# alibaba/EasyRec

Hardware: NVIDIA H100
Metric: samples_per_sec (higher is better)
Workload: dtype f32

## Files before the change

### easyrec_b200/csrc/embedding_bwd.cu

```cuda
#include "common.cuh"
#include "scan.cuh"
#include "slots.cuh"
#include "sort.cuh"
#include "bucket_bwd.cuh"

namespace er {

struct CBufs {
  const float* p[ER_MAX_BUFS];
};

constexpr int kLongRun = 64;
constexpr int kBatch = 4;
constexpr int kChunk = 512;

struct BwdArgs {
  float* table;
  float* state0;
  float* state1;
  int dim;
  int row_stride;
  uint32_t sentinel;
  const uint32_t* keys;
  const uint32_t* vals;
  const uint64_t* pairs;
  int64_t n;
  const float* weights;
  const int32_t* seg_ids;
  const er_slot_t* slots;
  int n_slots;
  CBufs gbufs;
  const float* seg_scale;
  er_opt_t opt;
  float lr_t;
  const float* hyper;
  int64_t* uniq_rows;
  float* uniq_grads;
  const int32_t* head_rank;
  int32_t* counters;
  int4* long_list;
  int32_t* run_done;
  int2* chunk_list;
  float* partials;
  const int64_t* or_rows;
  float* or_partials;
  int32_t* or_tickets;
  int or_chunks;
  int main_ctas;
};

__device__ __forceinline__ const float* grad_src(const BwdArgs& a, const SlotView& sv, uint32_t l,
                                                 float* coef) {
  const int32_t s = a.seg_ids ? a.seg_ids[l] : (int32_t)l;
  const SlotLite sl = slot_lite(sv, slot_of(sv, s));
  float c = (a.weights && !slot_unit_weights(sl)) ? a.weights[l] : 1.0f;
  if (a.seg_scale) c = __fmul_rn(c, a.seg_scale[s]);
  *coef = c;
  return a.gbufs.p[sl.misc & 0xff] + (int64_t)(s - sl.seg_begin) * sl.out_stride + sl.out_col;
}

struct Hyper {
  float lr, lr_t, grad_scale;
};

__device__ __forceinline__ Hyper load_hyper(const er_opt_t& o, float lr_t_arg, const float* __restrict__ hyper) {
  Hyper h;
  if (hyper) {
    h.lr = __ldg(hyper + ER_HYPER_LR);
    h.grad_scale = __ldg(hyper + ER_HYPER_GRAD_SCALE);
    h.lr_t = h.lr;
    if (o.kind == ER_OPT_LAZY_ADAM || o.kind == ER_OPT_ADAM_ROWS)
      h.lr_t = adam_lr_t_of(h.lr, __ldg(hyper + ER_HYPER_BETA1_POWER), __ldg(hyper + ER_HYPER_BETA2_POWER));
  } else {
    h.lr = o.lr;
    h.lr_t = lr_t_arg;
    h.grad_scale = o.grad_scale;
  }
  return h;
}

__device__ __forceinline__ void upd_one(const BwdArgs& a, const Hyper& h, float g, float& w, float& s0, float& s1) {
  switch (a.opt.kind) {
    case ER_OPT_ADAGRAD: {
      s0 = __fadd_rn(s0, __fmul_rn(g, g));
      w = __fsub_rn(w, __fmul_rn(__fmul_rn(h.lr, g), __frsqrt_rn(s0)));
      break;
    }
    case ER_OPT_LAZY_ADAM:
    case ER_OPT_ADAM_ROWS: {
      s0 = __fadd_rn(__fmul_rn(g, 1.0f - a.opt.beta1), __fmul_rn(s0, a.opt.beta1));
      s1 = __fadd_rn(__fmul_rn(__fmul_rn(g, g), 1.0f - a.opt.beta2), __fmul_rn(s1, a.opt.beta2));
      w = __fadd_rn(w, __fdiv_rn(__fmul_rn(-h.lr_t, s0), __fadd_rn(__fsqrt_rn(s1), a.opt.eps)));
      break;
    }
    case ER_OPT_MOMENTUM: {
      s0 = __fadd_rn(__fmul_rn(s0, a.opt.beta1), g);
      w = __fsub_rn(w, __fmul_rn(h.lr, s0));
      break;
    }
    default:
      w = __fsub_rn(w, __fmul_rn(h.lr, g));
  }
}

__device__ __forceinline__ void f4_fma_sep(float4& g, const float4& v, float c) {
  g.x = __fadd_rn(g.x, __fmul_rn(v.x, c));
  g.y = __fadd_rn(g.y, __fmul_rn(v.y, c));
  g.z = __fadd_rn(g.z, __fmul_rn(v.z, c));
  g.w = __fadd_rn(g.w, __fmul_rn(v.w, c));
}
__device__ __forceinline__ void f4_acc(float4& g, const float4& v) {
  g.x = __fadd_rn(g.x, v.x);
  g.y = __fadd_rn(g.y, v.y);
  g.z = __fadd_rn(g.z, v.z);
  g.w = __fadd_rn(g.w, v.w);
}

__device__ __forceinline__ float4 f4_scale1(const float4& v, float c) {
  return make_float4(__fmul_rn(v.x, c), __fmul_rn(v.y, c), __fmul_rn(v.z, c), __fmul_rn(v.w, c));
}

struct RowRegs {
  float4 w, s0, s1;
};

__device__ __forceinline__ RowRegs load_row(const BwdArgs& a, uint32_t row, int lane) {
  RowRegs r;
  r.w = r.s0 = r.s1 = make_float4(0.f, 0.f, 0.f, 0.f);
  if (!a.table) return r;
  const int64_t off = (int64_t)row * a.row_stride;
  r.w = reinterpret_cast<const float4*>(a.table + off)[lane];
  if (a.state0) r.s0 = reinterpret_cast<const float4*>(a.state0 + off)[lane];
  if (a.state1) r.s1 = reinterpret_cast<const float4*>(a.state1 + off)[lane];
  return r;
}

__device__ __forceinline__ void apply_row_vec(const BwdArgs& a, uint32_t row, int lane, float4 g,
                                              int64_t head_pos, RowRegs r) {
  const Hyper h = load_hyper(a.opt, a.lr_t, a.hyper);
  g.x = __fmul_rn(g.x, h.grad_scale);
  g.y = __fmul_rn(g.y, h.grad_scale);
  g.z = __fmul_rn(g.z, h.grad_scale);
  g.w = __fmul_rn(g.w, h.grad_scale);
  if (a.uniq_rows) {
    const int32_t u = a.head_rank[head_pos];
    if (lane == 0) a.uniq_rows[u] = (int64_t)row;
    reinterpret_cast<float4*>(a.uniq_grads + (int64_t)u * a.dim)[lane] = g;
  }
  if (!a.table) return;
  upd_one(a, h, g.x, r.w.x, r.s0.x, r.s1.x);
  upd_one(a, h, g.y, r.w.y, r.s0.y, r.s1.y);
  upd_one(a, h, g.z, r.w.z, r.s0.z, r.s1.z);
  upd_one(a, h, g.w, r.w.w, r.s0.w, r.s1.w);
  const int64_t off = (int64_t)row * a.row_stride;
  reinterpret_cast<float4*>(a.table + off)[lane] = r.w;
  if (a.state0) reinterpret_cast<float4*>(a.state0 + off)[lane] = r.s0;
  if (a.state1) reinterpret_cast<float4*>(a.state1 + off)[lane] = r.s1;
}

__device__ __forceinline__ void apply_scalar(const BwdArgs& a, uint32_t key, int c, float g,
                                             int64_t head_pos) {
  const Hyper h = load_hyper(a.opt, a.lr_t, a.hyper);
  g = __fmul_rn(g, h.grad_scale);
  if (a.uniq_rows) {
    const int32_t u = a.head_rank[head_pos];
    if (c == 0) a.uniq_rows[u] = (int64_t)key;
    a.uniq_grads[(int64_t)u * a.dim + c] = g;
  }
  if (!a.table) return;
  const int64_t off = (int64_t)key * a.row_stride + c;
  float w = a.table[off];
  float s0 = a.state0 ? a.state0[off] : 0.f;
  float s1 = a.state1 ? a.state1[off] : 0.f;
  upd_one(a, h, g, w, s0, s1);
  a.table[off] = w;
  if (a.state0) a.state0[off] = s0;
  if (a.state1) a.state1[off] = s1;
}

__device__ __forceinline__ int64_t run_end(const uint32_t* __restrict__ keys, int64_t lo, int64_t n,
                                           uint32_t key) {
  int64_t step = 1, hi = lo + 1;
  while (hi < n && keys[hi] == key) {
    lo = hi;
    step <<= 1;
    hi = lo + step;
  }
  if (hi > n) hi = n;
  while (hi - lo > 1) {
    const int64_t mid = (lo + hi) >> 1;
    if (keys[mid] == key)
      lo = mid;
    else
      hi = mid;
  }
  return hi;
}

__device__ __forceinline__ void enqueue_run(const BwdArgs& a, int64_t start, int len) {
  const int nch = (len + kChunk - 1) / kChunk;
  const int q = atomicAdd(&a.counters[0], 1);
  const int c0 = atomicAdd(&a.counters[1], nch);
  a.long_list[q] = make_int4((int)start, len, c0, nch);
  a.run_done[q] = 0;
  for (int c = 0; c < nch; ++c) a.chunk_list[c0 + c] = make_int2(q, c);
}

__device__ __forceinline__ void enqueue_long(const BwdArgs& a, int64_t start, int64_t j, uint32_t key) {
  enqueue_run(a, start, (int)(run_end(a.keys, j, a.n, key) - start));
}

__shared__ __align__(16) float s_or_part[1024];
__shared__ int s_or_last;
__shared__ long long s_or_row;

__device__ __forceinline__ int64_t one_row_row(const BwdArgs& a, const er_slot_t& sl) {
  for (int base = 0; base < sl.n_seg; base += blockDim.x) {
    const int e = base + threadIdx.x;
    const int64_t r = e < sl.n_seg ? a.or_rows[(int64_t)sl.seg_begin + e] : -1;
    if (threadIdx.x == 0) s_or_row = -1;
    __syncthreads();
    if (r >= 0) s_or_row = r;
    if (__syncthreads_or(r >= 0)) return s_or_row;
  }
  return -1;
}

template <int LANES>
__device__ __forceinline__ void one_row_cta(const BwdArgs& a, int cta) {
  const int f = cta / a.or_chunks, c_first = cta - f * a.or_chunks;
  const er_slot_t sl = a.slots[f];
  if (sl.bucket_mode != ER_BUCKET_ONE_ROW) return;
  constexpr int L = LANES > 0 ? LANES : 1;
  constexpr int G = 256 / L;
  const int dim = a.dim;
  const int used_chunks = (sl.n_seg + bk::kOneRowChunk - 1) / bk::kOneRowChunk;
  if (c_first >= used_chunks) return;
  const int used_ctas = min(a.or_chunks, used_chunks);
  float* const parts = a.or_partials + ((int64_t)f + sl.seg_begin / bk::kOneRowChunk) * dim;
  const float* gbuf = a.gbufs.p[sl.out_buf];
  if constexpr (LANES > 0) {
    const int grp = threadIdx.x / LANES, lane = threadIdx.x % LANES;
    float4 tot = make_float4(0.f, 0.f, 0.f, 0.f);
    for (int c = c_first; c < used_chunks; c += a.or_chunks) {
      const int s0 = c * bk::kOneRowChunk, s1 = min(sl.n_seg, s0 + bk::kOneRowChunk);
      float4 g = make_float4(0.f, 0.f, 0.f, 0.f);
      constexpr int U = 4;
      for (int e = s0 + grp; e < s1; e += G * U) {
        float4 v[U];
        float coef[U];
        bool use[U];
#pragma unroll
        for (int u = 0; u < U; ++u) {
          const int ee = e + u * G;
          use[u] = false;
          if (ee < s1) {
            const int64_t l = (int64_t)sl.seg_begin + ee;
            use[u] = a.or_rows[l] >= 0;
            coef[u] = a.weights ? a.weights[l] : 1.0f;
            if (a.seg_scale) coef[u] = __fmul_rn(coef[u], a.seg_scale[l]);
            v[u] = reinterpret_cast<const float4*>(gbuf + (int64_t)ee * sl.out_stride + sl.out_col)[lane];
          }
        }
#pragma unroll
        for (int u = 0; u < U; ++u)
          if (use[u]) f4_fma_sep(g, v[u], coef[u]);
      }
      reinterpret_cast<float4*>(s_or_part)[grp * LANES + lane] = g;
      __syncthreads();
      tot = make_float4(0.f, 0.f, 0.f, 0.f);
      if (threadIdx.x < LANES) {
        for (int q = 0; q < G; ++q) f4_acc(tot, reinterpret_cast<float4*>(s_or_part)[q * LANES + threadIdx.x]);
        __stcg(reinterpret_cast<float4*>(parts + (int64_t)c * dim) + threadIdx.x, tot);
      }
      __syncthreads();
    }
    __threadfence();
    __syncthreads();
    if (threadIdx.x == 0) s_or_last = (atomicAdd(&a.or_tickets[f], 1) == used_ctas - 1);
    __syncthreads();
    if (s_or_last) {
      __threadfence();
      for (int base = 0; base < used_chunks; base += G) {
        const int q = base + grp;
        if (q < used_chunks)
          reinterpret_cast<float4*>(s_or_part)[grp * LANES + lane] =
              __ldcg(reinterpret_cast<const float4*>(parts + (int64_t)q * dim) + lane);
        __syncthreads();
        if (threadIdx.x < LANES) {
          if (base == 0) tot = make_float4(0.f, 0.f, 0.f, 0.f);
          const int m = min(G, used_chunks - base);
          for (int q2 = 0; q2 < m; ++q2) f4_acc(tot, reinterpret_cast<float4*>(s_or_part)[q2 * LANES + threadIdx.x]);
        }
        __syncthreads();
      }
      const int64_t row = one_row_row(a, sl);
      if (threadIdx.x < LANES && row >= 0) {
        RowRegs r = load_row(a, (uint32_t)row, threadIdx.x);
        apply_row_vec(a, (uint32_t)row, threadIdx.x, tot, 0, r);
      }
      if (threadIdx.x == 0) a.or_tickets[f] = 0;
    }
  } else {
    for (int c = c_first; c < used_chunks; c += a.or_chunks) {
      const int s0 = c * bk::kOneRowChunk, s1 = min(sl.n_seg, s0 + bk::kOneRowChunk);
      for (int col = 0; col < dim; ++col) {
        float g = 0.f;
        for (int e = s0 + threadIdx.x; e < s1; e += 256) {
          const int64_t l = (int64_t)sl.seg_begin + e;
          if (a.or_rows[l] < 0) continue;
          float coef = a.weights ? a.weights[l] : 1.0f;
          if (a.seg_scale) coef = __fmul_rn(coef, a.seg_scale[l]);
          g = __fadd_rn(g, __fmul_rn(gbuf[(int64_t)e * sl.out_stride + sl.out_col + col], coef));
        }
        s_or_part[threadIdx.x] = g;
        __syncthreads();
        if (threadIdx.x == 0) {
          float tot = 0.f;
          for (int q = 0; q < 256; ++q) tot = __fadd_rn(tot, s_or_part[q]);
          __stcg(parts + (int64_t)c * dim + col, tot);
        }
        __syncthreads();
      }
    }
    __threadfence();
    __syncthreads();
    if (threadIdx.x == 0) s_or_last = (atomicAdd(&a.or_tickets[f], 1) == used_ctas - 1);
    __syncthreads();
    if (s_or_last) {
      __threadfence();
// ... 543 lines not shown
  row.w = row.s0 = row.s1 = make_float4(0.f, 0.f, 0.f, 0.f);
  if (r < R) row = load_row(a, (uint32_t)(sp[s_start[r]] >> 32), lane);
  float4 acc = make_float4(0.f, 0.f, 0.f, 0.f);
  for (int c0 = 0; c0 < n; c0 += S_ENT) {
    const int c1 = min(n, c0 + S_ENT);
    for (int q = threadIdx.x; q < (c1 - c0) * LANES; q += THREADS) {
      const int e = q / LANES;
      const uint32_t pos = (uint32_t)sp[c0 + e];
      if (pos != kDonePos) {
        float coef;
        const float* src = grad_src(a, sv, pos, &coef);
        s_stage[q] = f4_scale1(reinterpret_cast<const float4*>(src)[q % LANES], coef);
      }
    }
    __syncthreads();
    while (r < R && (int)s_start[r] < c1) {
      const int st = s_start[r], en = s_start[r + 1];
      const int lo = max(st, c0), hi = min(en, c1);
      for (int i = lo; i < hi; ++i) f4_acc(acc, s_stage[(i - c0) * LANES + lane]);
      if (en > c1) break;
      const uint32_t key = (uint32_t)(sp[st] >> 32);
      int rn = r + G;
      while (rn < R && run_is_long(s_start, rn)) rn += G;
      RowRegs nxt;
      nxt.w = nxt.s0 = nxt.s1 = make_float4(0.f, 0.f, 0.f, 0.f);
      if (rn < R) nxt = load_row(a, (uint32_t)(sp[s_start[rn]] >> 32), lane);
      apply_row_vec(a, key, lane, acc, 0, row);
      acc = make_float4(0.f, 0.f, 0.f, 0.f);
      row = nxt;
      r = rn;
    }
    __syncthreads();
  }
}

template <int THREADS, typename IdxT>
__device__ __forceinline__ void process_runs_scalar(const BwdArgs& a, const SlotView& sv, uint64_t* sp,
                                                    const IdxT* s_start, int R, float* s_stagef, float* s_partf,
                                                    int* s_coop, int* s_ncoop, int64_t queue_base) {
  const int dim = a.dim;
  if (threadIdx.x == 0) *s_ncoop = 0;
  __syncthreads();
  for (int r = threadIdx.x; r < R; r += THREADS)
    if (run_is_long(s_start, r)) s_coop[atomicAdd(s_ncoop, 1)] = r;
  __syncthreads();
  const int nco = *s_ncoop;
  for (int cc = 0; cc < nco; ++cc) {
    const int r = s_coop[cc];
    const int st = s_start[r], en = s_start[r + 1], len = en - st;
    if (queue_base >= 0 && len > bk::kQueueRun) {
      if (threadIdx.x == 0) enqueue_run(a, queue_base + st, len);
    } else {
      const int chunk = (len + THREADS - 1) / THREADS;
      const int j0 = st + threadIdx.x * chunk, j1 = min(en, j0 + chunk);
      const int used = (len + chunk - 1) / chunk;
      for (int c = 0; c < dim; ++c) {
        float g = 0.f;
        for (int j = j0; j < j1; ++j) {
          float coef;
          const float* src = grad_src(a, sv, (uint32_t)sp[j], &coef);
          g = __fadd_rn(g, __fmul_rn(src[c], coef));
        }
        s_partf[threadIdx.x] = g;
        __syncthreads();
        if (threadIdx.x == 0) {
          float tot = 0.f;
          for (int q = 0; q < used; ++q) tot = __fadd_rn(tot, s_partf[q]);
          apply_scalar(a, (uint32_t)(sp[st] >> 32), c, tot, 0);
        }
        __syncthreads();
      }
    }
    __syncthreads();
    for (int i = st + threadIdx.x; i < en; i += THREADS) sp[i] |= (uint64_t)kDonePos;
  }
  __syncthreads();
  const int n = s_start[R];
  const int S_ENT = max(1, (kStageF4 * 4) / dim);
  for (int cb = 0; cb < dim; cb += THREADS) {
    const int width = min(THREADS, dim - cb);
    const int total = R * width;
    int idx = threadIdx.x;
    float acc = 0.f;
    for (int c0 = 0; c0 < n; c0 += S_ENT) {
      const int c1 = min(n, c0 + S_ENT);
      for (int q = threadIdx.x; q < (c1 - c0) * dim; q += THREADS) {
        const int e = q / dim;
        const uint32_t pos = (uint32_t)sp[c0 + e];
        if (pos != kDonePos) {
          float coef;
          const float* src = grad_src(a, sv, pos, &coef);
          s_stagef[q] = __fmul_rn(src[q - e * dim], coef);
        }
      }
      __syncthreads();
      while (idx < total) {
        const int r = idx / width, c = cb + idx - r * width;
        if (run_is_long(s_start, r)) {
          idx += THREADS;
          continue;
        }
        const int st = s_start[r], en = s_start[r + 1];
        if (st >= c1) break;
        const int lo = max(st, c0), hi = min(en, c1);
        for (int i = lo; i < hi; ++i) acc = __fadd_rn(acc, s_stagef[(i - c0) * dim + c]);
        if (en > c1) break;
        apply_scalar(a, (uint32_t)(sp[st] >> 32), c, acc, 0);
        acc = 0.f;
        idx += THREADS;
      }
      __syncthreads();
    }
  }
}

inline size_t bk_reduce_smem(int n_slots, int cap, int threads) {
  return ((slot_smem_bytes(n_slots) + 15) & ~(size_t)15) + (size_t)cap * 8 + (((size_t)(cap + 1) * 2 + 15) & ~(size_t)15) +
         (size_t)max(kStageF4, threads) * 16 + (size_t)(cap / bk::kCoopRun + 2) * 4 + 64;
}

struct BkSmem {
  uint64_t* pairs;
  uint16_t* start;
  float4* stage;
  float4* part;
  int* coop;
  int* ncoop;
};
__device__ __forceinline__ BkSmem bk_carve(unsigned char* s_raw, int n_slots, int cap, int threads) {
  BkSmem m;
  unsigned char* p = s_raw + ((slot_smem_bytes(n_slots) + 15) & ~(size_t)15);
  m.pairs = reinterpret_cast<uint64_t*>(p); p += (size_t)cap * 8;
  m.start = reinterpret_cast<uint16_t*>(p); p += ((size_t)(cap + 1) * 2 + 15) & ~(size_t)15;
  m.stage = reinterpret_cast<float4*>(p); p += (size_t)max(kStageF4, threads) * 16;
  m.part = m.stage;
  m.coop = reinterpret_cast<int*>(p); p += (size_t)(cap / bk::kCoopRun + 1) * 4;
  m.ncoop = reinterpret_cast<int*>(p);
  return m;
}

__device__ __forceinline__ void cx(uint64_t& lo, uint64_t& hi, bool up) {
  if ((lo > hi) == up) {
    const uint64_t t = lo;
    lo = hi;
    hi = t;
  }
}

template <int LANES>
struct WarpSmem {
  float4 stage[32 * LANES];
  float4 carry[LANES];
  uint32_t keys[32];
};

__device__ __forceinline__ void sort4(uint64_t (&x)[4], int P, int lane) {
  for (int kk = 2; kk <= P; kk <<= 1) {
    for (int j = kk >> 1; j > 0; j >>= 1) {
      if (j == 64) {
        cx(x[0], x[2], ((lane) & kk) == 0);
        cx(x[1], x[3], ((lane + 32) & kk) == 0);
      } else if (j == 32) {
        cx(x[0], x[1], ((lane) & kk) == 0);
        if (P > 64) cx(x[2], x[3], ((lane + 64) & kk) == 0);
      } else {
        const bool lower = (lane & j) == 0;
#pragma unroll
        for (int r = 0; r < 4; ++r) {
          if (r * 32 < P) {
            const uint64_t other = __shfl_xor_sync(0xffffffffu, x[r], j);
            const bool up = ((lane + 32 * r) & kk) == 0;
            if ((x[r] > other) == (lower == up)) x[r] = other;
          }
        }
      }
    }
  }
}

template <int LANES>
__device__ __forceinline__ void warp_bucket_vec(const BwdArgs& a, const SlotView& sv, const BkArgs& k, int b,
                                                WarpSmem<LANES>* ws) {
  constexpr int G = 32 / LANES;
  const int lane = threadIdx.x & 31;
  const int gi = lane / LANES, gl = lane % LANES;
  const int n = k.w.bcnt[b];
  if (n == 0 || n > bk::kWarpCap) return;
  const int64_t off = k.w.boff[b];
  uint64_t x[4];
#pragma unroll
  for (int r = 0; r < 4; ++r) {
    const int q = r * 32 + lane;
    x[r] = q < n ? k.w.pairs[off + q] : ~0ull;
  }
  sort4(x, n <= 32 ? 32 : (n <= 64 ? 64 : 128), lane);
  uint32_t carry_key = 0xFFFFFFFFu;
#pragma unroll
  for (int r = 0; r < 4; ++r) {
    if (r * 32 >= n) break;
    const uint32_t key = (uint32_t)(x[r] >> 32), pos = (uint32_t)x[r];
    const int nv = min(32, n - r * 32);
    const uint32_t next_first = (r < 3 && (r + 1) * 32 < n) ? __shfl_sync(0xffffffffu, (uint32_t)(x[r < 3 ? r + 1 : 3] >> 32), 0)
                                                            : 0xFFFFFFFFu;
    uint32_t prevk = __shfl_up_sync(0xffffffffu, key, 1);
    if (lane == 0) prevk = carry_key;
    const bool is_head = lane < nv && key != prevk;
    const unsigned H = __ballot_sync(0xffffffffu, is_head);
    const int nh = __popc(H);
    ws->keys[lane] = key;
    const float4 open_sum = ws->carry[gl];
    RowRegs row0, row1;
    row0.w = row0.s0 = row0.s1 = row1.w = row1.s0 = row1.s1 = make_float4(0.f, 0.f, 0.f, 0.f);
    {
      const unsigned h0 = __fns(H, 0, gi + 1), h1 = __fns(H, 0, gi + G + 1);
      const uint32_t k0 = __shfl_sync(0xffffffffu, key, h0 & 31), k1 = __shfl_sync(0xffffffffu, key, h1 & 31);
      if (gi < nh) row0 = load_row(a, k0, gl);
      if (gi + G < nh) row1 = load_row(a, k1, gl);
    }
#pragma unroll
    for (int t = 0; t < LANES; ++t) {
      const int e = t * G + gi;
      const uint32_t pe = __shfl_sync(0xffffffffu, pos, e);
      if (e < nv) {
        float coef;
        const float* src = grad_src(a, sv, pe, &coef);
        ws->stage[e * LANES + gl] = f4_scale1(reinterpret_cast<const float4*>(src)[gl], coef);
      }
    }
    __syncwarp();
    const uint32_t lastk = ws->keys[31];
    const bool chunk_open = (nv == 32) && next_first == lastk;
    const int lead = nh ? (__ffs(H) - 1) : nv;
    if (lead > 0 && gi == 0) {
      float4 acc = open_sum;
      for (int i = 0; i < lead; ++i) f4_acc(acc, ws->stage[i * LANES + gl]);
      if (lead == 32 && chunk_open) {
        ws->carry[gl] = acc;
      } else {
        RowRegs row = load_row(a, carry_key, gl);
        apply_row_vec(a, carry_key, gl, acc, 0, row);
      }
    }
    for (int q = gi; q < nh; q += G) {
      const int h = __fns(H, 0, q + 1);
      const unsigned rest = (h == 31) ? 0u : (H >> (h + 1)) << (h + 1);
      const int e_end = rest ? (__ffs(rest) - 1) : nv;
      const uint32_t kh = ws->keys[h];
      float4 acc = make_float4(0.f, 0.f, 0.f, 0.f);
      for (int i = h; i < e_end; ++i) f4_acc(acc, ws->stage[i * LANES + gl]);
      if (e_end == 32 && chunk_open) {
        ws->carry[gl] = acc;
      } else {
        RowRegs row = (q == gi) ? row0 : (q == gi + G) ? row1 : load_row(a, kh, gl);
        apply_row_vec(a, kh, gl, acc, 0, row);
      }
    }
    carry_key = chunk_open ? lastk : 0xFFFFFFFFu;
    __syncwarp();
  }
}

struct WarpSmem1 {
  float stage[32];
  float carry;
  uint32_t keys[32];
};

__device__ __forceinline__ void warp_bucket_scalar(const BwdArgs& a, const SlotView& sv, const BkArgs& k, int b,
                                                   WarpSmem1* ws) {
  const int lane = threadIdx.x & 31;
  const int n = k.w.bcnt[b];
  if (n == 0 || n > bk::kWarpCap) return;
  const int64_t off = k.w.boff[b];
  uint64_t x[4];
#pragma unroll
  for (int r = 0; r < 4; ++r) {
    const int q = r * 32 + lane;
    x[r] = q < n ? k.w.pairs[off + q] : ~0ull;
  }
  sort4(x, n <= 32 ? 32 : (n <= 64 ? 64 : 128), lane);
#pragma unroll 1
  for (int col = 0; col < a.dim; ++col) {
    uint32_t carry_key = 0xFFFFFFFFu;
#pragma unroll
    for (int r = 0; r < 4; ++r) {
      if (r * 32 >= n) break;
      const uint32_t key = (uint32_t)(x[r] >> 32), pos = (uint32_t)x[r];
      const int nv = min(32, n - r * 32);
      const uint32_t next_first = (r < 3 && (r + 1) * 32 < n) ? __shfl_sync(0xffffffffu, (uint32_t)(x[r < 3 ? r + 1 : 3] >> 32), 0)
                                                              : 0xFFFFFFFFu;
      uint32_t prevk = __shfl_up_sync(0xffffffffu, key, 1);
      if (lane == 0) prevk = carry_key;
      const bool is_head = lane < nv && key != prevk;
      const unsigned H = __ballot_sync(0xffffffffu, is_head);
      const int nh = __popc(H);
      ws->keys[lane] = key;
      const float open_sum = ws->carry;
      if (lane < nv) {
        float coef;
        const float* src = grad_src(a, sv, pos, &coef);
        ws->stage[lane] = __fmul_rn(src[col], coef);
      }
      __syncwarp();
      const uint32_t lastk = ws->keys[31];
      const bool chunk_open = (nv == 32) && next_first == lastk;
      const int lead = nh ? (__ffs(H) - 1) : nv;
      if (lead > 0 && lane == 31) {
        float acc = open_sum;
        for (int i = 0; i < lead; ++i) acc = __fadd_rn(acc, ws->stage[i]);
        if (lead == 32 && chunk_open)
          ws->carry = acc;
        else
          apply_scalar(a, carry_key, col, acc, 0);
      }
      if (lane < nh && !(lead > 0 && lane == 31)) {
        const int h = __fns(H, 0, lane + 1);
        const unsigned rest = (h == 31) ? 0u : (H >> (h + 1)) << (h + 1);
        const int e_end = rest ? (__ffs(rest) - 1) : nv;
        float acc = 0.f;
        for (int i = h; i < e_end; ++i) acc = __fadd_rn(acc, ws->stage[i]);
        if (e_end == 32 && chunk_open)
          ws->carry = acc;
        else
          apply_scalar(a, ws->keys[h], col, acc, 0);
      }
      carry_key = chunk_open ? lastk : 0xFFFFFFFFu;
      __syncwarp();
    }
  }
}

constexpr bool warp_mode_lanes(int lanes) { return lanes == 1 || lanes == 2 || lanes == 4 || lanes == 8; }

template <int LANES>
inline size_t bk_fused_smem(int n_slots, bool warp_mode) {
  size_t warp_bytes = 0;
  if (warp_mode) {
    if constexpr (LANES > 0)
      warp_bytes = ((slot_smem_bytes(n_slots) + 15) & ~(size_t)15) + 8 * sizeof(WarpSmem<(LANES > 0 && LANES <= 8) ? LANES : 1>);
    else
      warp_bytes = ((slot_smem_bytes(n_slots) + 15) & ~(size_t)15) + 8 * sizeof(WarpSmem1);
  }
  const size_t med = bk_reduce_smem(n_slots, bk::kCap, bk::kThreads);
  return warp_bytes > med ? warp_bytes : med;
}

template <int LANES>
__global__ void __launch_bounds__(bk::kThreads, ER_BK_MINB) bk_fused_kernel(const __grid_constant__ BwdArgs a,
                                                                const __grid_constant__ BkArgs k) {
  extern __shared__ __align__(16) unsigned char s_raw[];
  __shared__ int s_warp[bk::kThreads / 32 + 1];
  const int bid = blockIdx.x;
  if (bid >= k.warp_ctas + k.med_ctas) {
    one_row_cta<LANES>(a, bid - k.warp_ctas - k.med_ctas);
    return;
  }
  const SlotView sv = load_slots(s_raw, a.slots, a.n_slots);
  if (bid < k.warp_ctas) {
    unsigned char* p = s_raw + ((slot_smem_bytes(a.n_slots) + 15) & ~(size_t)15);
    const int b = bid * 8 + (threadIdx.x >> 5);
    if constexpr (LANES > 0 && LANES <= 8) {
      warp_bucket_vec<LANES>(a, sv, k, b, reinterpret_cast<WarpSmem<LANES>*>(p) + (threadIdx.x >> 5));
    } else if constexpr (LANES == 0) {
      warp_bucket_scalar(a, sv, k, b, reinterpret_cast<WarpSmem1*>(p) + (threadIdx.x >> 5));
    }
    return;
  }
  const BkSmem m = bk_carve(s_raw, a.n_slots, bk::kCap, bk::kThreads);
  const int n_med = k.w.n_big[1];
  for (int xi = bid - k.warp_ctas; xi < n_med; xi += k.med_ctas) {
    const int b = k.w.med_list[xi];
    const int n = k.w.bcnt[b];
    const int off = k.w.boff[b];
    int P = 32;
    while (P < n) P <<= 1;
    for (int i = threadIdx.x; i < P; i += bk::kThreads) m.pairs[i] = i < n ? k.w.pairs[off + i] : ~0ull;
    __syncthreads();
    bk::bitonic_sort<bk::kThreads>(m.pairs, P);
    const int R = bk::run_starts<bk::kThreads, bk::kCap / bk::kThreads>(m.pairs, n, m.start, s_warp);
    if constexpr (LANES > 0)
      process_runs_vec<LANES, bk::kThreads>(a, sv, m.pairs, m.start, R, m.stage, m.part, m.coop, m.ncoop, -1);
    else
      process_runs_scalar<bk::kThreads>(a, sv, m.pairs, m.start, R, reinterpret_cast<float*>(m.stage),
                                        reinterpret_cast<float*>(m.part), m.coop, m.ncoop, -1);
    __syncthreads();
  }
}

__device__ __forceinline__ bool cta_radix_pass(const uint64_t* __restrict__ in, uint64_t* __restrict__ out, int n,
                                               int shift, int* s_wh , int* s_cur ) {
  const int lane = threadIdx.x & 31, wid = threadIdx.x >> 5;
  const unsigned lt_mask = (1u << lane) - 1u;
  for (int i = threadIdx.x; i < 256; i += bk::kBigThreads) s_cur[i] = 0;
  __syncthreads();
  for (int i = threadIdx.x; i < n; i += bk::kBigThreads) atomicAdd(&s_cur[(int)((in[i] >> shift) & 255)], 1);
  __syncthreads();
  int single = 0;
  if (threadIdx.x < 256) single = (s_cur[threadIdx.x] == n);
  if (__syncthreads_or(single)) return false;
  if (threadIdx.x < 32) {
    int carry = 0;
    for (int base = 0; base < 256; base += 32) {
      const int v = s_cur[base + lane];
      int incl = v;
#pragma unroll
      for (int o = 1; o < 32; o <<= 1) {
        const int t = __shfl_up_sync(0xffffffffu, incl, o);
        if (lane >= o) incl += t;
      }
      s_cur[base + lane] = carry + incl - v;
      carry += __shfl_sync(0xffffffffu, incl, 31);
    }
  }
  __syncthreads();
  for (int base = 0; base < n; base += bk::kBigThreads) {
    for (int i = threadIdx.x; i < 32 * 256; i += bk::kBigThreads) s_wh[i] = 0;
    __syncthreads();
    const int i = base + threadIdx.x;
    const bool valid = i < n;
    const uint64_t e = valid ? in[i] : 0ull;
    const int d = (int)((e >> shift) & 255);
    const unsigned peers = __match_any_sync(0xffffffffu, valid ? d : (256 + lane));
    const int r = __popc(peers & lt_mask);
    if (valid && r == 0) s_wh[wid * 256 + d] = __popc(peers);
    __syncthreads();
    if (threadIdx.x < 256) {
      int run = s_cur[threadIdx.x];
      for (int ww = 0; ww < 32; ++ww) {
        const int t = s_wh[ww * 256 + threadIdx.x];
        s_wh[ww * 256 + threadIdx.x] = run;
        run += t;
      }
      s_cur[threadIdx.x] = run;
    }
    __syncthreads();
    if (valid) out[s_wh[wid * 256 + d] + r] = e;
    __syncthreads();
  }
  return true;
}

template <int LANES>
__global__ void __launch_bounds__(bk::kBigThreads) bk_reduce_big_kernel(const __grid_constant__ BwdArgs a,
                                                                        const __grid_constant__ BkArgs k) {
  extern __shared__ __align__(16) unsigned char s_raw[];
  __shared__ int s_warp[bk::kBigThreads / 32 + 1];
  __shared__ int s_flag;
  const int n_big = k.w.n_big[0];
  if ((int)blockIdx.x >= n_big) return;
  const SlotView sv = load_slots(s_raw, a.slots, a.n_slots);
  const BkSmem m = bk_carve(s_raw, a.n_slots, bk::kBigCap, bk::kBigThreads);
  for (int x = blockIdx.x; x < n_big; x += gridDim.x) {
    const int b = k.w.big_list[x];
    const int n = k.w.bcnt[b];
    const int64_t off = k.w.boff[b];
    uint64_t* gp = k.w.pairs + off;
    bool sorted_in_global = false;
    if (n > bk::kBigCap) {
      int* s_wh = reinterpret_cast<int*>(m.pairs);
      int* s_cur = s_wh + 32 * 256;
      uint64_t* src = gp;
      uint64_t* dst = k.w.pairs_tmp + off;
      for (int shift = 0; shift < 64; shift += 8) {
        if (cta_radix_pass(src, dst, n, shift, s_wh, s_cur)) {
          uint64_t* t = src; src = dst; dst = t;
        }
        __syncthreads();
      }
      if (src != gp) {
        for (int i = threadIdx.x; i < n; i += bk::kBigThreads) gp[i] = src[i];
      }
      __threadfence_block();
      __syncthreads();
      sorted_in_global = true;
    }
    int p = 0;
    while (p < n) {
      const int mwin = min(bk::kBigCap, n - p);
      if (!sorted_in_global) {
        int P = 32;
        while (P < mwin) P <<= 1;
        for (int i = threadIdx.x; i < P; i += bk::kBigThreads) m.pairs[i] = i < mwin ? gp[i] : ~0ull;
        __syncthreads();
        bk::bitonic_sort<bk::kBigThreads>(m.pairs, P);
      } else {
        for (int i = threadIdx.x; i < mwin; i += bk::kBigThreads) m.pairs[i] = gp[p + i];
        __syncthreads();
      }
      int R = bk::run_starts<bk::kBigThreads, bk::kBigCap / bk::kBigThreads>(m.pairs, mwin, m.start, s_warp);
      int advance = mwin;
      if (sorted_in_global && p + mwin < n &&
          (uint32_t)(m.pairs[mwin - 1] >> 32) == (uint32_t)(gp[p + mwin] >> 32)) {
        if (R == 1) {
          const uint32_t key = (uint32_t)(m.pairs[0] >> 32);
          int lo = p + mwin, hi = n;
          while (lo < hi) {
            const int mid = (lo + hi) >> 1;
            if ((uint32_t)(gp[mid] >> 32) <= key) lo = mid + 1; else hi = mid;
          }
          if (threadIdx.x == 0) enqueue_run(a, off + p, lo - p);
          p = lo;
          __syncthreads();
          continue;
        }
        advance = m.start[R - 1];
        R -= 1;
      }
      if (!sorted_in_global) {
        if (threadIdx.x == 0) s_flag = 0;
        __syncthreads();
        for (int r = threadIdx.x; r < R; r += bk::kBigThreads)
          if (m.start[r + 1] - m.start[r] > bk::kQueueRun) s_flag = 1;
        __syncthreads();
        if (s_flag)
          for (int i = threadIdx.x; i < mwin; i += bk::kBigThreads) gp[i] = m.pairs[i];
      }
      if constexpr (LANES > 0)
        process_runs_vec<LANES, bk::kBigThreads>(a, sv, m.pairs, m.start, R, m.stage, m.part, m.coop, m.ncoop, off + p);
      else
        process_runs_scalar<bk::kBigThreads>(a, sv, m.pairs, m.start, R, reinterpret_cast<float*>(m.stage),
                                             reinterpret_cast<float*>(m.part), m.coop, m.ncoop, off + p);
      p += advance;
      __syncthreads();
    }
  }
}

struct HeadIn {
  const uint32_t* keys;
  uint32_t sentinel;
  __device__ int operator()(int64_t j) const {
    uint32_t k = keys[j];
    return (k < sentinel && (j == 0 || keys[j - 1] != k)) ? 1 : 0;
  }
};
struct HeadOut {
  int32_t* rank;
  __device__ void operator()(int64_t j, int ex, int) const { rank[j] = ex; }
};

inline size_t a256(size_t x) { return (x + 255) & ~(size_t)255; }

struct BwdWs {
  uint32_t* keys;
  uint32_t* vals;
  int32_t* head_rank;
  int4* long_list;
  int32_t* run_done;
  int2* chunk_list;
  float* partials;
  int32_t* counters;
  void* sort_ws;
  void* scan_ws;
  bk::Ws bk;
  int32_t* tickets;
  float* one_row_partials;
};

inline int64_t max_long_runs(int64_t n) { return n / kLongRun + 1; }
inline int64_t max_chunks(int64_t n) { return n / kChunk + max_long_runs(n) + 1; }
inline int64_t max_one_row_parts(int64_t n) { return n / bk::kOneRowChunk + 2048 + 1; }

inline BwdWs bwd_carve(void* ws, int64_t n, int dim, char** end = nullptr) {
  char* p = reinterpret_cast<char*>(a256(reinterpret_cast<size_t>(ws)));
  BwdWs w;
  w.keys = reinterpret_cast<uint32_t*>(p); p += a256((size_t)n * 4);
  w.vals = reinterpret_cast<uint32_t*>(p); p += a256((size_t)n * 4);
  w.head_rank = reinterpret_cast<int32_t*>(p); p += a256((size_t)n * 4);
  w.long_list = reinterpret_cast<int4*>(p); p += a256((size_t)max_long_runs(n) * 16);
  w.run_done = reinterpret_cast<int32_t*>(p); p += a256((size_t)max_long_runs(n) * 4);
  w.chunk_list = reinterpret_cast<int2*>(p); p += a256((size_t)max_chunks(n) * 8);
  w.partials = reinterpret_cast<float*>(p); p += a256((size_t)max_chunks(n) * dim * 4);
  w.bk = bk::carve(p, n, &w.counters, &w.tickets, &p);
  w.one_row_partials = reinterpret_cast<float*>(p); p += a256((size_t)max_one_row_parts(n) * dim * 4);
  w.sort_ws = p; p += a256(rsort::workspace_bytes(n));
  w.scan_ws = p; p += a256(scan::workspace_bytes(n));
  if (end) *end = p;
  return w;
}

inline size_t bwd_ws_bytes(int64_t n, int dim) {
  char* end;
  bwd_carve(nullptr, n, dim, &end);
  return reinterpret_cast<size_t>(end) + 768;
}

static float adam_lr_t(const er_opt_t& o) { return adam_lr_t_of(o.lr, o.beta1_power, o.beta2_power); }

template <int LANES>
static void launch_long(const BwdArgs& a, cudaStream_t st) {
  const size_t sl = slot_smem_bytes(a.n_slots);
  if constexpr (LANES > 0) {
    constexpr int TPE = (LANES <= 8) ? 1 : LANES;
    const size_t smem_long = ((sl + 15) & ~(size_t)15) + (size_t)8 * LANES * sizeof(float4);
    bwd_long_vec_kernel<LANES, TPE><<<4 * kSmCount, 256, smem_long, st>>>(a);
  } else {
    bwd_long_scalar_kernel<<<4 * kSmCount, 256, sl, st>>>(a);
  }
}

template <int LANES>
static void launch_radix(const BwdArgs& a, cudaStream_t st) {
  const size_t smem = slot_smem_bytes(a.n_slots);
  const unsigned grid = (unsigned)ceil_div(a.n, 256);
  if constexpr (LANES > 8) {
    bwd_runs_vec_kernel<LANES><<<grid, 256, smem, st>>>(a);
  } else if constexpr (LANES > 0) {
    const size_t smem_scan = ((smem + 15) & ~(size_t)15) + (size_t)8 * 32 * LANES * sizeof(float4);
    bwd_scan_vec_kernel<LANES><<<grid, 256, smem_scan, st>>>(a);
  } else if (a.dim == 1) {
    bwd_scan_d1_kernel<<<grid, 256, smem, st>>>(a);
  } else {
    bwd_runs_scalar_kernel<<<(unsigned)ceil_div(a.n * a.dim, 256), 256, smem, st>>>(a);
  }
  launch_long<LANES>(a, st);
  count_launches(2);
}

static int log2_of(int v) {
  int l = 0;
  while ((1 << l) < v) ++l;
  return l;
}

static bool k7_warp_mode(int dim) { return dim == 1 || dim == 4 || dim == 8 || dim == 16 || dim == 32; }

static void bk_place(const int64_t* rows, int64_t cap, const int32_t* n_dev, int64_t n_rows, const int32_t* seg_ids,
                     const er_slot_t* slots, int n_slots, bool one_row, bool warp_mode, const BwdWs& w,
                     bool zero_call_block, cudaStream_t st) {
  bk::PlaceArgs pa;
  pa.rows = rows;
  pa.cap = cap;
  pa.n_dev = n_dev;
  pa.sentinel = (uint32_t)n_rows;
  pa.seg_ids = seg_ids;
  pa.slots = one_row ? slots : nullptr;
  pa.n_slots = n_slots;
  const int nb = bk::num_buckets(cap, warp_mode);
  pa.log2_nb = log2_of(nb);
  pa.warp_cap = warp_mode ? bk::kWarpCap : 0;
  pa.w = w.bk;
  cudaMemsetAsync(w.bk.bcnt, 0, bk::zero_place_bytes() + (zero_call_block ? bk::zero_call_bytes() : 0), st);
  const size_t smem = bk::place_smem_bytes(n_slots, nb, pa.slots != nullptr);
  static bool attr = false;
  if (!attr) {
    const int mx = (int)bk::place_smem_bytes(2048, bk::kMaxBuckets, true);
    cudaFuncSetAttribute(bk::bk_count_kernel, cudaFuncAttributeMaxDynamicSharedMemorySize, mx);
    cudaFuncSetAttribute(bk::bk_place_kernel, cudaFuncAttributeMaxDynamicSharedMemorySize, mx);
    attr = true;
  }
  const unsigned tiles = (unsigned)ceil_div(cap, (int64_t)bk::kTile);
  bk::bk_count_kernel<<<tiles, bk::kTileThreads, smem, st>>>(pa);
  bk::bk_place_kernel<<<tiles, bk::kTileThreads, smem, st>>>(pa);
  count_launches(2);
}

template <int LANES>
static void bk_launch_fused(BwdArgs a, const BwdWs& place, bool place_warp_mode, cudaStream_t st) {
  BkArgs k;
  k.w = place.bk;
  const int nb = bk::num_buckets(a.n, place_warp_mode);
  k.log2_nb = log2_of(nb);
  k.warp_ctas = place_warp_mode ? (nb >> 3) : 0;
  k.med_ctas = place_warp_mode ? kSmCount : nb;
  const size_t smem = bk_fused_smem<LANES>(a.n_slots, place_warp_mode);
  const size_t smem_big = bk_reduce_smem(a.n_slots, bk::kBigCap, bk::kBigThreads);
  static bool attr = false;
  if (!attr) {
    cudaFuncSetAttribute(bk_fused_kernel<LANES>, cudaFuncAttributeMaxDynamicSharedMemorySize,
                         (int)bk_fused_smem<LANES>(2048, true));
    cudaFuncSetAttribute(bk_fused_kernel<LANES>, cudaFuncAttributePreferredSharedMemoryCarveout,
                         (int)cudaSharedmemCarveoutMaxShared);
    cudaFuncSetAttribute(bk_reduce_big_kernel<LANES>, cudaFuncAttributeMaxDynamicSharedMemorySize,
                         (int)bk_reduce_smem(2048, bk::kBigCap, bk::kBigThreads));
    attr = true;
  }
  const int extra = a.or_chunks * a.n_slots;
  a.main_ctas = k.warp_ctas + k.med_ctas;
  bk_fused_kernel<LANES><<<k.warp_ctas + k.med_ctas + extra, bk::kThreads, smem, st>>>(a, k);
  bk_reduce_big_kernel<LANES><<<kSmCount, bk::kBigThreads, smem_big, st>>>(a, k);
  launch_long<LANES>(a, st);
  count_launches(3);
}

}

extern "C" size_t er_sort_workspace_bytes(int64_t n) { return er::rsort::workspace_bytes(n > 0 ? n : 1); }

extern "C" int er_sort_rows(const int64_t* rows, int64_t n, const int32_t* n_dev, int64_t max_row,
                            uint32_t* keys_out, uint32_t* vals_out, void* ws, size_t ws_bytes,
                            er_stream_t stream) {
  using namespace er;
  ER_REQUIRE(rows && keys_out && vals_out, "null argument");
  ER_REQUIRE(n > 0 && n < (1LL << 31), "n out of range");
  ER_REQUIRE(max_row > 0 && max_row < 0xFFFFFFFFLL, "max_row must be in (0, 2^32-1)");
  if (!ws || ws_bytes < rsort::workspace_bytes(n))
    return fail(ER_ERR_WORKSPACE, "er_sort_rows: workspace too small");
  rsort::sort_rows(rows, n, n_dev, max_row, keys_out, vals_out, ws, nullptr, as_stream(stream));
  ER_CUDA_LAUNCH_CHECK();
  return ER_OK;
}

extern "C" size_t er_embedding_bwd_workspace_bytes(int64_t n_lookups_cap, int32_t dim) {
  return er::bwd_ws_bytes(n_lookups_cap > 0 ? n_lookups_cap : 1, dim > 0 ? dim : 1);
}

static int embedding_bwd_impl(float* table, float* state0, float* state1, int64_t n_rows,
                              int32_t dim, int32_t row_stride, const int64_t* rows,
                              const float* weights, const int32_t* seg_ids,
                              const int32_t* row_ptr, int64_t n_seg, int64_t n_lookups_cap,
                              const er_slot_t* slots, int32_t n_slots,
                              const float* const* grad_bufs, int32_t n_bufs,
                              const float* seg_scale, const er_opt_t* opt, int64_t* uniq_rows,
                              float* uniq_grads, int32_t* n_uniq, void* ws, size_t ws_bytes,
                              const void* sorted_ws, size_t sorted_ws_bytes, int32_t sorted_dim,
                              er_stream_t stream) {
  using namespace er;
  ER_REQUIRE(rows && slots && grad_bufs && opt, "null argument");
  ER_REQUIRE(table || uniq_rows, "nothing to do: table and uniq_rows are both NULL");
  ER_REQUIRE((uniq_rows == nullptr) == (uniq_grads == nullptr) &&
                 (uniq_rows == nullptr) == (n_uniq == nullptr),
             "uniq_rows, uniq_grads and n_uniq go together");
  ER_REQUIRE(dim > 0 && row_stride >= dim, "bad dim / row_stride");
  ER_REQUIRE(dim <= kStageF4 * 4, "dim must be at most 4096");
  ER_REQUIRE(n_rows > 0 && n_rows < 0xFFFFFFFFLL, "n_rows must be in (0, 2^32-1)");
  ER_REQUIRE(n_slots > 0 && n_slots <= 2048, "n_slots must be in [1, 2048]");
  ER_REQUIRE(n_bufs > 0 && n_bufs <= ER_MAX_BUFS, "n_bufs must be in [1, ER_MAX_BUFS]");
  ER_REQUIRE(n_lookups_cap >= 0 && n_lookups_cap < (1LL << 31), "n_lookups_cap out of range");
  ER_REQUIRE(row_ptr || seg_ids || n_lookups_cap == n_seg,
             "without row_ptr / seg_ids every segment must hold exactly one lookup");
  ER_REQUIRE(!row_ptr || seg_ids, "CSR input needs seg_ids (er_csr_from_lens)");
  if (table) {
    const int k = opt->kind;
    ER_REQUIRE(k == ER_OPT_SGD || k == ER_OPT_ADAGRAD || k == ER_OPT_LAZY_ADAM || k == ER_OPT_ADAM_ROWS || k == ER_OPT_MOMENTUM,
               "unknown optimizer kind");
    ER_REQUIRE(k == ER_OPT_SGD || state0, "optimizer state0 missing");
    ER_REQUIRE((k != ER_OPT_LAZY_ADAM && k != ER_OPT_ADAM_ROWS) || state1, "adam needs state1 (v)");
  }
  if (n_lookups_cap == 0) return ER_OK;
  if (!ws || ws_bytes < bwd_ws_bytes(n_lookups_cap, dim))
    return fail(ER_ERR_WORKSPACE, "er_embedding_bwd: workspace too small");
  cudaStream_t st = as_stream(stream);
  BwdWs w = bwd_carve(ws, n_lookups_cap, dim);
  const int32_t* n_dev = row_ptr ? row_ptr + n_seg : nullptr;
  const bool bucketed = (uniq_rows == nullptr);
  const bool one_row = bucketed && seg_ids == nullptr;
  BwdWs src = w;
  if (sorted_ws) {
    if (sorted_ws_bytes < bwd_ws_bytes(n_lookups_cap, sorted_dim))
      return fail(ER_ERR_WORKSPACE, "er_embedding_bwd_reuse_sort: source workspace too small");
    if (!bucketed)
      return fail(ER_ERR_UNSUPPORTED, "er_embedding_bwd_reuse_sort: uniq_rows output needs the rows (er_embedding_bwd)");
    if (k7_warp_mode(sorted_dim) != k7_warp_mode(dim))
      return fail(ER_ERR_UNSUPPORTED, "er_embedding_bwd_reuse_sort: the placement was made in the other placement mode "
                                      "(warp-sized buckets for dims 1, 4, 8, 16 and 32, CTA-sized for the others)");
    src = bwd_carve(const_cast<void*>(sorted_ws), n_lookups_cap, sorted_dim);
    cudaMemsetAsync(w.counters, 0, bk::zero_call_bytes(), st);
  } else if (bucketed) {
    bk_place(rows, n_lookups_cap, n_dev, n_rows, seg_ids, slots, n_slots, one_row, k7_warp_mode(dim), w, true, st);
  } else {
    rsort::sort_rows(rows, n_lookups_cap, n_dev, n_rows, w.keys, w.vals, w.sort_ws, w.counters, st);
  }
  const bool place_warp = k7_warp_mode(dim);

  BwdArgs a = {};
  a.table = table;
  a.state0 = state0;
  a.state1 = state1;
  a.dim = dim;
  a.row_stride = row_stride;
  a.sentinel = (uint32_t)n_rows;
  a.keys = w.keys;
  a.vals = w.vals;
  a.pairs = nullptr;
  a.n = n_lookups_cap;
  a.weights = weights;
  a.seg_ids = seg_ids;
  a.slots = slots;
  a.n_slots = n_slots;
  bool aligned = true;
  for (int i = 0; i < ER_MAX_BUFS; ++i) {
    a.gbufs.p[i] = i < n_bufs ? grad_bufs[i] : nullptr;
    if (i < n_bufs) {
      ER_REQUIRE(grad_bufs[i] != nullptr, "null gradient buffer");
      aligned = aligned && (reinterpret_cast<uintptr_t>(grad_bufs[i]) % 16 == 0);
    }
  }
  a.seg_scale = seg_scale;
  a.opt = *opt;
  a.lr_t = (opt->kind == ER_OPT_LAZY_ADAM || opt->kind == ER_OPT_ADAM_ROWS) ? adam_lr_t(*opt) : opt->lr;
  a.hyper = opt->hyper_dev;
  a.uniq_rows = uniq_rows;
  a.uniq_grads = uniq_grads;
  a.head_rank = nullptr;
  a.counters = w.counters;
  a.long_list = w.long_list;
  a.run_done = w.run_done;
  a.chunk_list = w.chunk_list;
  a.partials = w.partials;
  a.or_rows = rows;
  a.or_partials = w.one_row_partials;
  a.or_tickets = w.tickets;
  a.or_chunks = one_row ? (int)ceil_div(ceil_div(n_lookups_cap, (int64_t)n_slots), (int64_t)bk::kOneRowChunk) : 0;
  if (uniq_rows) {
    scan::exclusive_scan(HeadIn{w.keys, a.sentinel}, HeadOut{w.head_rank}, n_lookups_cap, n_uniq,
                         w.scan_ws, st);
    a.head_rank = w.head_rank;
    count_launches(3);
  }
  if (table) {
    aligned = aligned && reinterpret_cast<uintptr_t>(table) % 16 == 0 && row_stride % 4 == 0 &&
              (!state0 || reinterpret_cast<uintptr_t>(state0) % 16 == 0) &&
              (!state1 || reinterpret_cast<uintptr_t>(state1) % 16 == 0);
  }
  if (uniq_grads) aligned = aligned && reinterpret_cast<uintptr_t>(uniq_grads) % 16 == 0;
  const bool vec_dim = (dim == 4 || dim == 8 || dim == 16 || dim == 32 || dim == 64 || dim == 128);
  if (bucketed) {
    ER_REQUIRE(table != nullptr, "the bucketed path updates a table");
    a.keys = nullptr;
    a.vals = nullptr;
    a.pairs = src.bk.pairs;
    if (vec_dim && aligned) {
      switch (dim / 4) {
// ... 231 lines not shown
```

Measured before the change: 11.05 million.

## Prefetch all run-head rows via cp.async and hoist scalar row loads

In the warp-per-bucket vector path, the weight and optimizer-state rows for every run head (and the carried run) are now fetched asynchronously into per-warp shared memory with cp.async. These copies overlap with gradient staging, replacing the earlier scheme that held only two rows in registers and did serial loads for the rest. The scalar path loads row state before the gradient gather and merges the carry and head branches. The CTA order is also swapped so medium-bucket CTAs come first, and the scalar kernel gets its own launch-bounds minimum. The per-warp shared memory footprint grows, which may reduce occupancy.

```diff
diff --git a/easyrec_b200/csrc/embedding_bwd.cu b/easyrec_b200/csrc/embedding_bwd.cu
--- a/easyrec_b200/csrc/embedding_bwd.cu
+++ b/easyrec_b200/csrc/embedding_bwd.cu
@@ -158,8 +158,22 @@
   if (a.state1) reinterpret_cast<float4*>(a.state1 + off)[lane] = r.s1;
 }
 
-__device__ __forceinline__ void apply_scalar(const BwdArgs& a, uint32_t key, int c, float g,
-                                             int64_t head_pos) {
+struct ScalarRow {
+  float w, s0, s1;
+};
+
+__device__ __forceinline__ ScalarRow load_scalar(const BwdArgs& a, uint32_t key, int c) {
+  ScalarRow r{0.f, 0.f, 0.f};
+  if (!a.table) return r;
+  const int64_t off = (int64_t)key * a.row_stride + c;
+  r.w = a.table[off];
+  if (a.state0) r.s0 = a.state0[off];
+  if (a.state1) r.s1 = a.state1[off];
+  return r;
+}
+
+__device__ __forceinline__ void apply_scalar(const BwdArgs& a, uint32_t key, int c, float g, int64_t head_pos,
+                                             ScalarRow r) {
   const Hyper h = load_hyper(a.opt, a.lr_t, a.hyper);
   g = __fmul_rn(g, h.grad_scale);
   if (a.uniq_rows) {
@@ -169,13 +183,15 @@
   }
   if (!a.table) return;
   const int64_t off = (int64_t)key * a.row_stride + c;
-  float w = a.table[off];
-  float s0 = a.state0 ? a.state0[off] : 0.f;
-  float s1 = a.state1 ? a.state1[off] : 0.f;
-  upd_one(a, h, g, w, s0, s1);
-  a.table[off] = w;
-  if (a.state0) a.state0[off] = s0;
-  if (a.state1) a.state1[off] = s1;
+  upd_one(a, h, g, r.w, r.s0, r.s1);
+  a.table[off] = r.w;
+  if (a.state0) a.state0[off] = r.s0;
+  if (a.state1) a.state1[off] = r.s1;
+}
+
+__device__ __forceinline__ void apply_scalar(const BwdArgs& a, uint32_t key, int c, float g,
+                                             int64_t head_pos) {
+  apply_scalar(a, key, c, g, head_pos, load_scalar(a, key, c));
 }
 
 __device__ __forceinline__ int64_t run_end(const uint32_t* __restrict__ keys, int64_t lo, int64_t n,
@@ -1025,7 +1041,20 @@
   float4 stage[32 * LANES];
   float4 carry[LANES];
   uint32_t keys[32];
+  float4 rows[33 * LANES];
 };
+
+template <int LANES>
+__host__ __device__ constexpr size_t warp_smem_bytes(int n_row_arrays) {
+  return sizeof(WarpSmem<LANES>) + (size_t)(n_row_arrays - 1) * 33 * LANES * sizeof(float4);
+}
+
+__device__ __forceinline__ void cp_async16(void* smem, const void* gmem) {
+  asm volatile("cp.async.cg.shared.global [%0], [%1], 16;\n" ::"r"((unsigned)__cvta_generic_to_shared(smem)),
+               "l"(gmem)
+               : "memory");
+}
+__device__ __forceinline__ void cp_async_wait_all() { asm volatile("cp.async.wait_all;\n" ::: "memory"); }
 
 __device__ __forceinline__ void sort4(uint64_t (&x)[4], int P, int lane) {
   for (int kk = 2; kk <= P; kk <<= 1) {
@@ -1055,11 +1084,15 @@
 __device__ __forceinline__ void warp_bucket_vec(const BwdArgs& a, const SlotView& sv, const BkArgs& k, int b,
                                                 WarpSmem<LANES>* ws) {
   constexpr int G = 32 / LANES;
+  constexpr int ROWS = 33 * LANES;
   const int lane = threadIdx.x & 31;
   const int gi = lane / LANES, gl = lane % LANES;
   const int n = k.w.bcnt[b];
   if (n == 0 || n > bk::kWarpCap) return;
   const int64_t off = k.w.boff[b];
+  float4* const rw = ws->rows;
+  float4* const r0 = rw + ROWS;
+  float4* const r1 = r0 + (a.state0 ? ROWS : 0);
   uint64_t x[4];
 #pragma unroll
   for (int r = 0; r < 4; ++r) {
@@ -1067,6 +1100,19 @@
     x[r] = q < n ? k.w.pairs[off + q] : ~0ull;
   }
   sort4(x, n <= 32 ? 32 : (n <= 64 ? 64 : 128), lane);
+  auto fetch = [&](uint32_t kh, int slot) {
+    const int64_t o = (int64_t)kh * a.row_stride + 4 * gl;
+    cp_async16(rw + slot * LANES + gl, a.table + o);
+    if (a.state0) cp_async16(r0 + slot * LANES + gl, a.state0 + o);
+    if (a.state1) cp_async16(r1 + slot * LANES + gl, a.state1 + o);
+  };
+  auto staged = [&](int slot) {
+    RowRegs row;
+    row.w = rw[slot * LANES + gl];
+    row.s0 = a.state0 ? r0[slot * LANES + gl] : make_float4(0.f, 0.f, 0.f, 0.f);
+    row.s1 = a.state1 ? r1[slot * LANES + gl] : make_float4(0.f, 0.f, 0.f, 0.f);
+    return row;
+  };
   uint32_t carry_key = 0xFFFFFFFFu;
 #pragma unroll
   for (int r = 0; r < 4; ++r) {
@@ -1080,15 +1126,16 @@
     const bool is_head = lane < nv && key != prevk;
     const unsigned H = __ballot_sync(0xffffffffu, is_head);
     const int nh = __popc(H);
+    const uint32_t lastk = __shfl_sync(0xffffffffu, key, 31);
+    const bool chunk_open = (nv == 32) && next_first == lastk;
+    const int lead = nh ? (__ffs(H) - 1) : nv;
     ws->keys[lane] = key;
     const float4 open_sum = ws->carry[gl];
-    RowRegs row0, row1;
-    row0.w = row0.s0 = row0.s1 = row1.w = row1.s0 = row1.s1 = make_float4(0.f, 0.f, 0.f, 0.f);
-    {
-      const unsigned h0 = __fns(H, 0, gi + 1), h1 = __fns(H, 0, gi + G + 1);
-      const uint32_t k0 = __shfl_sync(0xffffffffu, key, h0 & 31), k1 = __shfl_sync(0xffffffffu, key, h1 & 31);
-      if (gi < nh) row0 = load_row(a, k0, gl);
-      if (gi + G < nh) row1 = load_row(a, k1, gl);
+    __syncwarp();
+    if (lead > 0 && gi == 0 && !(lead == 32 && chunk_open)) fetch(carry_key, 32);
+    for (int q = gi; q < nh; q += G) {
+      const int h = __fns(H, 0, q + 1);
+      if (!(chunk_open && h == 31 - __clz(H))) fetch(ws->keys[h], q);
     }
 #pragma unroll
     for (int t = 0; t < LANES; ++t) {
@@ -1100,19 +1147,15 @@
         ws->stage[e * LANES + gl] = f4_scale1(reinterpret_cast<const float4*>(src)[gl], coef);
       }
     }
+    cp_async_wait_all();
     __syncwarp();
-    const uint32_t lastk = ws->keys[31];
-    const bool chunk_open = (nv == 32) && next_first == lastk;
-    const int lead = nh ? (__ffs(H) - 1) : nv;
     if (lead > 0 && gi == 0) {
       float4 acc = open_sum;
       for (int i = 0; i < lead; ++i) f4_acc(acc, ws->stage[i * LANES + gl]);
-      if (lead == 32 && chunk_open) {
+      if (lead == 32 && chunk_open)
         ws->carry[gl] = acc;
-      } else {
-        RowRegs row = load_row(a, carry_key, gl);
-        apply_row_vec(a, carry_key, gl, acc, 0, row);
-      }
+      else
+        apply_row_vec(a, carry_key, gl, acc, 0, staged(32));
     }
     for (int q = gi; q < nh; q += G) {
       const int h = __fns(H, 0, q + 1);
@@ -1121,12 +1164,10 @@
       const uint32_t kh = ws->keys[h];
       float4 acc = make_float4(0.f, 0.f, 0.f, 0.f);
       for (int i = h; i < e_end; ++i) f4_acc(acc, ws->stage[i * LANES + gl]);
-      if (e_end == 32 && chunk_open) {
+      if (e_end == 32 && chunk_open)
         ws->carry[gl] = acc;
-      } else {
-        RowRegs row = (q == gi) ? row0 : (q == gi + G) ? row1 : load_row(a, kh, gl);
-        apply_row_vec(a, kh, gl, acc, 0, row);
-      }
+      else
+        apply_row_vec(a, kh, gl, acc, 0, staged(q));
     }
     carry_key = chunk_open ? lastk : 0xFFFFFFFFu;
     __syncwarp();
@@ -1167,6 +1208,19 @@
       const bool is_head = lane < nv && key != prevk;
       const unsigned H = __ballot_sync(0xffffffffu, is_head);
       const int nh = __popc(H);
+      const uint32_t lastk = __shfl_sync(0xffffffffu, key, 31);
+      const bool chunk_open = (nv == 32) && next_first == lastk;
+      const int lead = nh ? (__ffs(H) - 1) : nv;
+      const bool carried = lead > 0 && lane == 31;
+      const int h = __fns(H, 0, lane + 1) & 31;
+      const uint32_t kh = __shfl_sync(0xffffffffu, key, h);
+      const unsigned rest = (h == 31) ? 0u : (H >> (h + 1)) << (h + 1);
+      const int e_end = rest ? (__ffs(rest) - 1) : nv;
+      const bool mine = carried || lane < nh;
+      const bool stays_open = carried ? (lead == 32 && chunk_open) : (e_end == 32 && chunk_open);
+      const uint32_t my_key = carried ? carry_key : kh;
+      ScalarRow row{0.f, 0.f, 0.f};
+      if (mine && !stays_open) row = load_scalar(a, my_key, col);
       ws->keys[lane] = key;
       const float open_sum = ws->carry;
       if (lane < nv) {
@@ -1175,27 +1229,13 @@
         ws->stage[lane] = __fmul_rn(src[col], coef);
       }
       __syncwarp();
-      const uint32_t lastk = ws->keys[31];
-      const bool chunk_open = (nv == 32) && next_first == lastk;
-      const int lead = nh ? (__ffs(H) - 1) : nv;
-      if (lead > 0 && lane == 31) {
-        float acc = open_sum;
-        for (int i = 0; i < lead; ++i) acc = __fadd_rn(acc, ws->stage[i]);
-        if (lead == 32 && chunk_open)
+      if (mine) {
+        float acc = carried ? open_sum : 0.f;
+        for (int i = carried ? 0 : h; i < (carried ? lead : e_end); ++i) acc = __fadd_rn(acc, ws->stage[i]);
+        if (stays_open)
           ws->carry = acc;
         else
-          apply_scalar(a, carry_key, col, acc, 0);
-      }
-      if (lane < nh && !(lead > 0 && lane == 31)) {
-        const int h = __fns(H, 0, lane + 1);
-        const unsigned rest = (h == 31) ? 0u : (H >> (h + 1)) << (h + 1);
-        const int e_end = rest ? (__ffs(rest) - 1) : nv;
-        float acc = 0.f;
-        for (int i = h; i < e_end; ++i) acc = __fadd_rn(acc, ws->stage[i]);
-        if (e_end == 32 && chunk_open)
-          ws->carry = acc;
-        else
-          apply_scalar(a, ws->keys[h], col, acc, 0);
+          apply_scalar(a, my_key, col, acc, 0, row);
       }
       carry_key = chunk_open ? lastk : 0xFFFFFFFFu;
       __syncwarp();
@@ -1206,11 +1246,12 @@
 constexpr bool warp_mode_lanes(int lanes) { return lanes == 1 || lanes == 2 || lanes == 4 || lanes == 8; }
 
 template <int LANES>
-inline size_t bk_fused_smem(int n_slots, bool warp_mode) {
+inline size_t bk_fused_smem(int n_slots, bool warp_mode, int n_row_arrays) {
   size_t warp_bytes = 0;
   if (warp_mode) {
     if constexpr (LANES > 0)
-      warp_bytes = ((slot_smem_bytes(n_slots) + 15) & ~(size_t)15) + 8 * sizeof(WarpSmem<(LANES > 0 && LANES <= 8) ? LANES : 1>);
+      warp_bytes = ((slot_smem_bytes(n_slots) + 15) & ~(size_t)15) +
+                   8 * warp_smem_bytes<(LANES > 0 && LANES <= 8) ? LANES : 1>(n_row_arrays);
     else
       warp_bytes = ((slot_smem_bytes(n_slots) + 15) & ~(size_t)15) + 8 * sizeof(WarpSmem1);
   }
@@ -1218,9 +1259,12 @@
   return warp_bytes > med ? warp_bytes : med;
 }
 
+#ifndef ER_BK_MINB_SCALAR
+#define ER_BK_MINB_SCALAR 5
+#endif
 template <int LANES>
-__global__ void __launch_bounds__(bk::kThreads, ER_BK_MINB) bk_fused_kernel(const __grid_constant__ BwdArgs a,
-                                                                const __grid_constant__ BkArgs k) {
+__global__ void __launch_bounds__(bk::kThreads, LANES == 0 ? ER_BK_MINB_SCALAR : ER_BK_MINB)
+    bk_fused_kernel(const __grid_constant__ BwdArgs a, const __grid_constant__ BkArgs k) {
   extern __shared__ __align__(16) unsigned char s_raw[];
   __shared__ int s_warp[bk::kThreads / 32 + 1];
   const int bid = blockIdx.x;
@@ -1229,11 +1273,13 @@
     return;
   }
   const SlotView sv = load_slots(s_raw, a.slots, a.n_slots);
-  if (bid < k.warp_ctas) {
+  if (bid >= k.med_ctas) {
     unsigned char* p = s_raw + ((slot_smem_bytes(a.n_slots) + 15) & ~(size_t)15);
-    const int b = bid * 8 + (threadIdx.x >> 5);
+    const int b = (bid - k.med_ctas) * 8 + (threadIdx.x >> 5);
     if constexpr (LANES > 0 && LANES <= 8) {
-      warp_bucket_vec<LANES>(a, sv, k, b, reinterpret_cast<WarpSmem<LANES>*>(p) + (threadIdx.x >> 5));
+      const int n_row_arrays = 1 + (a.state0 != nullptr) + (a.state1 != nullptr);
+      warp_bucket_vec<LANES>(
+          a, sv, k, b, reinterpret_cast<WarpSmem<LANES>*>(p + (threadIdx.x >> 5) * warp_smem_bytes<LANES>(n_row_arrays)));
     } else if constexpr (LANES == 0) {
       warp_bucket_scalar(a, sv, k, b, reinterpret_cast<WarpSmem1*>(p) + (threadIdx.x >> 5));
     }
@@ -1241,7 +1287,7 @@
   }
   const BkSmem m = bk_carve(s_raw, a.n_slots, bk::kCap, bk::kThreads);
   const int n_med = k.w.n_big[1];
-  for (int xi = bid - k.warp_ctas; xi < n_med; xi += k.med_ctas) {
+  for (int xi = bid; xi < n_med; xi += k.med_ctas) {
     const int b = k.w.med_list[xi];
     const int n = k.w.bcnt[b];
     const int off = k.w.boff[b];
@@ -1536,12 +1582,12 @@
   k.log2_nb = log2_of(nb);
   k.warp_ctas = place_warp_mode ? (nb >> 3) : 0;
   k.med_ctas = place_warp_mode ? kSmCount : nb;
-  const size_t smem = bk_fused_smem<LANES>(a.n_slots, place_warp_mode);
+  const size_t smem = bk_fused_smem<LANES>(a.n_slots, place_warp_mode, 1 + (a.state0 != nullptr) + (a.state1 != nullptr));
   const size_t smem_big = bk_reduce_smem(a.n_slots, bk::kBigCap, bk::kBigThreads);
   static bool attr = false;
   if (!attr) {
     cudaFuncSetAttribute(bk_fused_kernel<LANES>, cudaFuncAttributeMaxDynamicSharedMemorySize,
-                         (int)bk_fused_smem<LANES>(2048, true));
+                         (int)bk_fused_smem<LANES>(2048, true, 3));
     cudaFuncSetAttribute(bk_fused_kernel<LANES>, cudaFuncAttributePreferredSharedMemoryCarveout,
                          (int)cudaSharedmemCarveoutMaxShared);
     cudaFuncSetAttribute(bk_reduce_big_kernel<LANES>, cudaFuncAttributeMaxDynamicSharedMemorySize,
```

New measurement: 11.24 million, median of 6. 1.02x the previous value.
